# wonheeML/mtl-ssl

Hardware: AMD Instinct MI355X
Metric: images/sec training, Faster R-CNN ResNet-101 + aux heads (higher is better)
Workload: dtype f32; 1 GPU; Faster R-CNN ResNet-101 + window/closeness/edgemask heads + refine, synthetic 1024x600 COCO-shaped (90 classes), per-GPU batch 2 (BASELINE.json configs[1]); global_batch=2, parallelism=dp1, pipeline_config=configs/frcnn_resnet101_coco_mtl.config

## Files before the change

### include/mtlssl_hip.h

```cpp
#ifndef MTLSSL_HIP_H_
#define MTLSSL_HIP_H_

#include <stdint.h>

#ifdef __cplusplus
extern "C" {
#endif

typedef void* mtlssl_stream_t;

#define MTLSSL_OK 0
#define MTLSSL_EINVAL (-1)
#define MTLSSL_ELAUNCH (-2)
#define MTLSSL_ECOMM (-3)

#define MTLSSL_ABI_VERSION 23

const char* mtlssl_last_error(void);
int mtlssl_abi_version(void);

int mtlssl_exp_rn(const double* x, double* y, int64_t n, mtlssl_stream_t stream);

typedef struct {
  int32_t N, H, W, C;
  int32_t K, R, S;
  int32_t OH, OW;
  int32_t stride, dilation;
  int32_t pad_t, pad_l;
  int32_t ldy;
} mtlssl_conv_desc;

#define MTLSSL_EPI_BIAS 1
#define MTLSSL_EPI_RESIDUAL 2
#define MTLSSL_EPI_RELU 4
#define MTLSSL_EPI_TANH 8
#define MTLSSL_EPI_RELU6 16
#define MTLSSL_EPI_MASK 32
#define MTLSSL_EPI_ACCUM 64
#define MTLSSL_EPI_MASK6 128

int64_t mtlssl_conv2d_workspace_bytes(const mtlssl_conv_desc* d, int mode);
int mtlssl_conv2d_fwd(const mtlssl_conv_desc* d, const float* x, const float* w,
                      const float* bias, const float* residual, float* y, int epilogue,
                      void* workspace, mtlssl_stream_t stream);
int mtlssl_conv2d_dgrad(const mtlssl_conv_desc* d, const float* dy, const float* w,
                        const float* residual, const float* mask_ref, float* dx, int epilogue,
                        void* workspace, mtlssl_stream_t stream);
int64_t mtlssl_conv2d_filter_xf_bytes(const mtlssl_conv_desc* d, int mode);
int mtlssl_conv2d_filter_xf_variant(const mtlssl_conv_desc* d, int mode);
// ... 18 lines not shown
typedef struct {
  const float* w;
  float* y;
  const float* bias;
  int32_t K, ldy, epilogue, reserved;
} mtlssl_conv_group_entry;
int mtlssl_conv2d_fwd_grouped(const mtlssl_conv_desc* d, const float* x, int n, const mtlssl_conv_group_entry* entries,
                              int max_k, int sum_k, mtlssl_stream_t stream);
typedef struct {
  const float* dy;
  const float* w;
  int32_t K, ldy;
} mtlssl_conv_seg_entry;
int mtlssl_conv2d_dgrad_segmented(const mtlssl_conv_desc* d, int n, const mtlssl_conv_seg_entry* entries,
                                  const float* residual, const float* mask_ref, float* dx, int epilogue,
                                  mtlssl_stream_t stream);
int mtlssl_conv2d_wgrad_ex(const mtlssl_conv_desc* d, const float* x, const float* dy,
                           const float* out_scale, float* dw, float* dbias, const float* dbias_scale, float beta,
                           void* workspace, const float* input_xf, int input_variant, mtlssl_stream_t stream);
int64_t mtlssl_conv2d_wgrad_workspace_bytes(const mtlssl_conv_desc* d);
int mtlssl_conv2d_tile_config(const mtlssl_conv_desc* d, int mode);
int mtlssl_conv2d_force_config(const mtlssl_conv_desc* d, int mode, int cfg);
int mtlssl_conv2d_set_winograd(int mode);
int mtlssl_conv2d_set_pointwise(int on);
int mtlssl_conv2d_dgrad_rs(const mtlssl_conv_desc* d, const float* dy, const float* w, const float* residual,
                           const float* mask_ref, float* dx, int epilogue, void* workspace, const float* filter_xf,
                           int xf_variant, const uint8_t* group_active, int rows_per_group, mtlssl_stream_t stream);
int mtlssl_conv2d_wgrad_rs(const mtlssl_conv_desc* d, const float* x, const float* dy,
                           const float* out_scale, float* dw, float* dbias, const float* dbias_scale, float beta,
                           void* workspace, const float* input_xf, int input_variant, const uint8_t* group_active,
                           int rows_per_group, mtlssl_stream_t stream);
int mtlssl_row_group_flags(const float* scale, int n, uint8_t* flags, mtlssl_stream_t stream);
int mtlssl_conv2d_set_row_skip(int on);
int mtlssl_conv2d_set_fp32_engine(int mode);
int mtlssl_conv2d_engine_launches(int64_t* out, int reset);
int mtlssl_conv2d_num_dispatches(const mtlssl_conv_desc* d, int mode);
#define MTLSSL_PLAN_INFO_LEN 16
#define MTLSSL_PLAN_DIRECT 0
#define MTLSSL_PLAN_PADDED 1
#define MTLSSL_PLAN_THIN 2
#define MTLSSL_PLAN_S2D 3
#define MTLSSL_PLAN_PARITY 4
#define MTLSSL_PLAN_WINO_F43 5
#define MTLSSL_PLAN_WINO_M7 6
#define MTLSSL_PLAN_VALU 7
int mtlssl_conv2d_plan_info(const mtlssl_conv_desc* d, int mode, int parity_class, int32_t* out);
int64_t mtlssl_conv2d_executed_macs(const mtlssl_conv_desc* d, int mode, int on_mfma);
int mtlssl_conv2d_wgrad(const mtlssl_conv_desc* d, const float* x, const float* dy,
                        const float* out_scale, float* dw, float* dbias, float beta,
                        void* workspace, mtlssl_stream_t stream);

int64_t mtlssl_conv2d_wgrad_grouped_workspace_bytes(const mtlssl_conv_desc* d, int n);
int mtlssl_conv2d_wgrad_grouped(const mtlssl_conv_desc* d, int n, const void* x_ptrs, const void* dy_ptrs,
                                const void* scale_ptrs, const void* dw_ptrs, float beta, void* workspace,
                                mtlssl_stream_t stream);

int mtlssl_depthwise_fwd(const mtlssl_conv_desc* d, const float* x, const float* w, const float* bias,
                         float* y, int epilogue, mtlssl_stream_t stream);
int mtlssl_depthwise_dgrad(const mtlssl_conv_desc* d, const float* dy, const float* w,
                           const float* mask_ref, float* dx, int epilogue, mtlssl_stream_t stream);
int64_t mtlssl_depthwise_wgrad_workspace_bytes(const mtlssl_conv_desc* d);
int mtlssl_depthwise_wgrad(const mtlssl_conv_desc* d, const float* x, const float* dy,
                           const float* out_scale, float* dw, float beta, void* workspace,
                           mtlssl_stream_t stream);
int64_t mtlssl_bn_param_grads_workspace_bytes(int C);
int mtlssl_bn_param_grads(const float* y, const float* g, const float* gamma, const float* beta,
// ... 285 lines not shown
```

### mtl_ssl_amd/build.py

```python
import hashlib
import os
import subprocess
import sys
from concurrent.futures import ThreadPoolExecutor

HERE = os.path.dirname(os.path.abspath(__file__))
CSRC = os.path.join(HERE, "csrc")
OUT = os.path.join(HERE, "libmtlssl_hip.so")
OBJ = os.path.join(HERE, "build")
HIPCC = os.environ.get("HIPCC", "/opt/rocm/bin/hipcc")
COMMON = ["--offload-arch=gfx950", "-O3", "-std=c++17", "-fPIC", "-Wno-unused-result"]
SOURCES = {
    "detection.hip": ["-ffp-contract=off"],
    "ops.hip": ["-ffp-contract=off"],
    "conv.hip": [],
    "glue.hip": ["-ffp-contract=off"],
    "depthwise.hip": [], "pool_concat.hip": [], "winograd.hip": [],
    "eval_metrics.hip": ["-ffp-contract=off"],
    "coco_eval.hip": ["-ffp-contract=off"],
    "pascal_eval.hip": ["-ffp-contract=off"],
    "aux_labels.hip": ["-ffp-contract=off"],
    "summaries.hip": ["-ffp-contract=off"],
    "batch_norm.hip": ["-ffp-contract=off", "-fhip-fp32-correctly-rounded-divide-sqrt"],
    "visualize.hip": [],
    "comm.hip": [],
}


def _digest(path, flags):
    h = hashlib.sha256()
    for f in (path, os.path.join(CSRC, "common.h"), os.path.join(CSRC, "conv_mfma.h"), os.path.join(CSRC, "conv_split.h"), os.path.join(CSRC, "portable_math.h"),
              os.path.join(HERE, "..", "include", "mtlssl_hip.h")):
        with open(f, "rb") as fh:
            h.update(fh.read())
    h.update(" ".join(flags).encode())
    return h.hexdigest()


def build(force=False, verbose=True):
    os.makedirs(OBJ, exist_ok=True)
    jobs, digests = [], []
    for src, extra in SOURCES.items():
        path = os.path.join(CSRC, src)
        obj = os.path.join(OBJ, src + ".o")
        stamp = obj + ".sha"
        dig = _digest(path, COMMON + extra)
        digests.append(dig)
        if (not force and os.path.exists(obj) and os.path.exists(stamp)
                and open(stamp).read() == dig):
            continue
        jobs.append((path, obj, stamp, dig, extra))
    link_stamp = os.path.join(OBJ, "link.sha")
    link_dig = hashlib.sha256("\n".join(digests).encode()).hexdigest()
    if not force and os.path.exists(OUT) and os.path.exists(link_stamp) and open(link_stamp).read() == link_dig:
        return OUT

    def run(job):
        path, obj, stamp, dig, extra = job
        cmd = [HIPCC] + COMMON + extra + ["-c", path, "-o", obj]
        if verbose:
            print(" ".join(cmd), flush=True)
        subprocess.check_call(cmd)
        with open(stamp, "w") as f:
            f.write(dig)
# ... 18 lines not shown
```

### mtl_ssl_amd/csrc/conv.hip

```cpp
#include <stdlib.h>

#include <atomic>
#include <mutex>
#include <unordered_map>

#include "conv_mfma.h"
#include "conv_split.h"

namespace mtlssl {

__global__ void __launch_bounds__(256) k_row_group_flags(const float* __restrict__ scale, int n, uint8_t* __restrict__ flags) {
  const int i = blockIdx.x * blockDim.x + threadIdx.x;
  if (i < n) flags[i] = scale[i] != 0.f;
}
__global__ void __launch_bounds__(256) k_active_ksteps(const uint8_t* __restrict__ flags, int rpg, int P, int pps, int stride,
                                                       int* __restrict__ out) {
  const int z = blockIdx.x, pix0 = z * pps, pix1 = min(P, pix0 + pps);
  const int ksteps = (max(pix1 - pix0, 0) + BK - 1) / BK;
  const int lane = threadIdx.x & 63, w = threadIdx.x >> 6;
  int* list = out + KSTEP_HDR + (int64_t)z * stride;
  __shared__ int wave_cnt[4];
  int base = 0;
  for (int s0 = 0; s0 < ksteps; s0 += 256) {
    const int s = s0 + threadIdx.x;
    bool act = false;
    if (s < ksteps) {
      const int r0 = pix0 + s * BK, r1 = min(r0 + BK, pix1) - 1;
      for (int g = r0 / rpg; g <= r1 / rpg; ++g) act |= flags[g] != 0;
    }
    const unsigned long long m = __ballot(act);
    if (lane == 0) wave_cnt[w] = __popcll(m);
    __syncthreads();
    int off = base;
    for (int i = 0; i < w; ++i) off += wave_cnt[i];
    if (act) list[off + __popcll(m & ((1ull << lane) - 1ull))] = s;
    base += wave_cnt[0] + wave_cnt[1] + wave_cnt[2] + wave_cnt[3];
    __syncthreads();
  }
  if (threadIdx.x == 0) out[z] = base;
}
static inline int64_t kstep_list_bytes(int64_t P) { return align_up((KSTEP_HDR + 2 * cdiv(P, BK) + 128) * 4, 256); }
static std::atomic<int>& row_skip_ref() { static std::atomic<int> v{1}; return v; }

__global__ void __launch_bounds__(256) k_wgrad_reduce(const float* ws, int nsplit, int64_t total4, int K,
                                                      const float* scale, float* dw, float beta, int main_blocks,
                                                      const float* cs_part, int cs_chunks, float* dbias,
                                                      const float* dbias_scale) {
  if ((int)blockIdx.x >= main_blocks) {
    const int lane = threadIdx.x & 63;
    const int k = ((int)blockIdx.x - main_blocks) * 4 + (threadIdx.x >> 6);
    if (k >= K) return;
    float s = 0.f;
    for (int c = lane; c < cs_chunks; c += 64) s += cs_part[(int64_t)c * K + k];
    s = wave_sum(s);
    if (dbias_scale) s *= dbias_scale[k];
    if (lane == 0) dbias[k] = beta != 0.f ? beta * dbias[k] + s : s;
    return;
  }
  const int64_t t = blockIdx.x * (int64_t)blockDim.x + threadIdx.x;
  const int64_t i = t >> 2;
  const int sl = (int)(t & 3);
  const bool live = i < total4;
  floatx4 s = {0.f, 0.f, 0.f, 0.f};
  if (live)
    for (int k = sl; k < nsplit; k += 4) s += reinterpret_cast<const floatx4*>(ws)[(int64_t)k * total4 + i];
#pragma unroll
  for (int e = 0; e < 4; ++e) {
    s[e] += __shfl_xor(s[e], 1, 64);
    s[e] += __shfl_xor(s[e], 2, 64);
  }
  if (!live || sl) return;
  if (scale) s *= *reinterpret_cast<const floatx4*>(scale + (i * 4) % K);
  floatx4* d = reinterpret_cast<floatx4*>(dw) + i;
  *d = beta != 0.f ? beta * *d + s : s;
}
// ... 1227 lines not shown
      (void)hipMemsetAsync(w_pad + (int64_t)d->C * d->K, 0, (size_t)(q.C - d->C) * d->K * 4, S(stream));
      launch_packed<MODE_FWD>(r, p, x_pad, w_pad, workspace, S(stream));
      break;
    }
    case FAM_THIN:
      hipLaunchKernelGGL(k_pw_thin_fwd, dim3(cdiv(p.M, 4)), dim3(256), 0, S(stream), x, w, bias, residual, y, p.M, d->C, d->K, epi);
      break;
    case FAM_GEMM_SMALL: {
      GemmArgs g{x, w, y, bias, residual, nullptr, p.M, d->K, d->C, epi, 0};
      hipLaunchKernelGGL(k_gemm_small<GM_FWD>, dim3(cdiv(g.N, 64), cdiv(g.M, 64)), dim3(256), 0, S(stream), g);
      break;
    }
    case FAM_S2D: {
      float* xs = (float*)workspace;
      float* wsf = (float*)((char*)workspace + r.front_a);
      hipLaunchKernelGGL(k_s2d_pack, dim3(cdiv((int64_t)q.N * q.H * q.W * 4, 256)), dim3(256), 0, S(stream), x, d->N, d->H, d->W,
                         d->C, d->pad_t, d->pad_l, q.H, q.W, xs);
      hipLaunchKernelGGL(k_s2d_filter, dim3(cdiv((int64_t)q.R * q.S * q.C * q.K, 256)), dim3(256), 0, S(stream), w, d->R, d->S,
                         d->C, d->K, q.R, q.S, wsf);
      launch_packed<MODE_FWD>(r, p, xs, wsf, workspace, S(stream));
      break;
    }
    case FAM_STEM_FWD: {
      dim3 grid(cdiv(d->OW, STEM_T), cdiv(d->OH, STEM_T), d->N);
      hipLaunchKernelGGL(k_conv_smallc_fwd, grid, dim3(256), stem_lds_bytes(d), S(stream), p);
      break;
    }
    default:
      hipLaunchKernelGGL(k_conv_direct_fwd, dim3(cdiv((int64_t)p.M * p.K, 256)), dim3(256), 0, S(stream), p);
  }
  return check_launch("conv2d_fwd");
}

int mtlssl_conv2d_fwd_grouped(const mtlssl_conv_desc* d, const float* x, int n, const mtlssl_conv_group_entry* entries,
                              int max_k, int sum_k, mtlssl_stream_t stream) {
  if (n <= 0) return MTLSSL_OK;
  if (int rc = check_desc(d)) return rc;
  MTLSSL_REQUIRE(is_pointwise(d) && d->dilation == 1, "fwd_grouped: pointwise problems only (1x1, stride 1, no padding)");
  MTLSSL_REQUIRE(d->C % BK == 0, "fwd_grouped: C = %d must be a multiple of %d", d->C, BK);
  MTLSSL_REQUIRE(x && entries && n <= MTLSSL_CONV_GROUP_MAX && max_k >= 16 && sum_k >= max_k, "fwd_grouped: bad arguments");
  ConvArgs p = make_args(d);
  GroupArgs ga;
  memset(&ga, 0, sizeof(ga));
  p.a = x;
  for (int i = 0; i < n; ++i) {
    const mtlssl_conv_group_entry& e = entries[i];
    MTLSSL_REQUIRE(e.w && e.y && e.K >= 16 && e.K % 4 == 0 && e.K <= max_k && (e.ldy == 0 || (e.ldy >= e.K && e.ldy % 4 == 0)) &&
                       !(e.epilogue & (MTLSSL_EPI_RESIDUAL | MASK_ANY | MTLSSL_EPI_ACCUM)) && (!(e.epilogue & MTLSSL_EPI_BIAS) || e.bias),
                   "fwd_grouped: problem %d: K = %d, ldy = %d, epilogue = %d", i, e.K, e.ldy, e.epilogue);
    ga.e[i] = e;
  }
  p.a_bytes = (unsigned)((int64_t)d->N * d->H * d->W * d->C * 4);
  p.M = d->N * d->H * d->W;
  p.NG = max_k; p.K = max_k; p.ldy = 0;
  p.nsplit = 1; p.ks_per_split = 0; p.tile_m0 = 0; p.ws_m0 = 0;
  int cfg = 2;
  double best = 1e30;
  for (int c = 0; c < NCFG; ++c) {
    const int64_t tiles = cdiv(p.M, CFG_BM[c]) * cdiv(sum_k, CFG_BN[c]);
    const double t = tile_time_us(c, tiles, d->C / CFG_BK[c], true);
    if (t < best) { best = t; cfg = c; }
  }
  p.tiles_m = (int)cdiv(p.M, CFG_BM[cfg]);
  p.tiles_n = (int)cdiv(max_k, CFG_BN[cfg]);
  dim3 grid(p.tiles_m * p.tiles_n, n, 1);
  count_engine_launch(0);
// ... 448 lines not shown
```

### mtl_ssl_amd/frcnn.py

```python
import os

import torch

from . import nn, ops

f32, i32 = torch.float32, torch.int32


def _init_from_hyperparams(hp):
    ini = hp.initializer
    which = ini.which_oneof(["truncated_normal_initializer", "variance_scaling_initializer"])
    if which == "truncated_normal_initializer":
        return ("truncated_normal", float(ini.truncated_normal_initializer.stddev))
    if which == "variance_scaling_initializer":
        v = ini.variance_scaling_initializer
        return ("variance_scaling", float(v.factor), str(v.mode), bool(v.uniform))
    return ("variance_scaling", 1.0, "FAN_AVG", True)


def _l2_from_hyperparams(hp):
    reg = hp.regularizer
    if reg.has("l2_regularizer"):
        return float(reg.l2_regularizer.weight)
    return 0.0
# ... 32 lines not shown
        if not self.spatial_average:
            if feat_hw is None:
                raise ValueError("mask_rcnn_box_predictor without spatial_average needs the tower's output size")
            width = cin * int(feat_hw[0]) * int(feat_hw[1])
        depth = max(min(cin, int(cfg.max_depth)), int(cfg.min_depth))
        self.stack = None
        n_extra = int(cfg.num_layers_before_predictor) if depth > 0 else 0
        if n_extra > 0:
            act = {"RELU": "relu", "NONE": None}.get(str(cfg.fc_hyperparams.activation))
            if act is None and str(cfg.fc_hyperparams.activation) != "NONE":
                raise ValueError("fc_hyperparams.activation %s is not supported in the predictor's extra layers"
                                 % cfg.fc_hyperparams.activation)
            self.stack = nn.FCStack(ps, ["%s/FC_%d_%d" % (scope, i, depth) for i in range(n_extra)], width,
                                    [depth] * n_extra, init, is_training, wd, activation=act,
                                    keep_prob=float(cfg.dropout_keep_probability) if cfg.use_dropout else None,
                                    slot0=slot0, batch_norm=bn)
            width = depth
        self.box = None
        if not class_only:
            self.box = nn.Conv(ps, scope + "/BoxEncodingPredictor", width, num_classes * 4, 1, init,
                               is_training, wd, fc=True, batch_norm=bn and bn())
            self.cls = nn.Conv(ps, scope + "/ClassPredictor", width, num_classes + 1, 1, init, is_training,
                               wd, fc=True, batch_norm=bn and bn())
        else:
            self.cls = nn.Conv(ps, scope + "/ClassPredictor", width, num_classes, 1, init, is_training, wd,
                               fc=True, batch_norm=bn and bn())

    def layers(self):
        extra = self.stack.layers if self.stack is not None else []
        return extra + [l for l in (self.box, self.cls) if l is not None]

    def predict(self, feat, seed=0, step=0, update=False):
        pooled = ops.spatial_mean_fwd(feat) if self.spatial_average else feat.reshape(feat.shape[0], -1)
        net, sctx = pooled, None
        if self.stack is not None:
            net, sctx = self.stack.forward(pooled, self.is_training, seed, step, update)
        out = {"pooled": net, "_stack_ctx": sctx}
        for key, head in (("class", self.cls), ("box", self.box)):
            if head is not None and head.batch_stats:
                keep = out["_norm_" + key] = {}
                out[key] = head.forward(net, keep, update)
            elif head is not None:
                out[key] = head.forward(net)
        return out

    def backward(self, pred, d_class, d_box, feat_shape, need_feat_grad=True, mask_ref=None, mask6=False):
        net = pred["pooled"]
        if self.cls.norm is not None:
            d_class = self.cls.norm_backward(pred.get("_norm_class"), pred["class"], d_class)
            if d_box is not None:
                d_box = self.box.norm_backward(pred.get("_norm_box"), pred["box"], d_box)
        self.cls.wgrad(net, d_class)
        if d_box is not None:
            self.box.wgrad(net, d_box)
        if not need_feat_grad and self.stack is None:
            return None
        dp = self.cls.dgrad(net.shape, d_class)
        if d_box is not None:
            self.box.dgrad(net.shape, d_box, out=dp, accum=True)
        if self.stack is not None:
            dp = self.stack.backward(pred["_stack_ctx"], dp, need_input_grad=need_feat_grad)
        if not need_feat_grad:
            return None
        if self.spatial_average:
            return ops.spatial_mean_bwd(dp, feat_shape, mask_ref, mask6)
        g = dp.reshape(tuple(feat_shape))
# ... 431 lines not shown
        stop = bool(self._mtl.stop_gradient_for_aux_tasks)
        need_crop_grad = not stop
        crops, argmax = self._crop(F, flat, box_ind, need_crop_grad)
        save = self._is_training and not (self._shared_classifier and stop)
        feat, ctx = self.window_tower.forward(crops, save)
        wp = self.window_predictor.predict(feat, self.seed, self.step)
        pd.update({"window_class_predictions": wp["class"], "_wfeat": feat, "_wctx": ctx, "_wp": wp,
                   "_wcrops": crops, "_wargmax": argmax, "_wboxes": flat, "_wbox_ind": box_ind})
        return pd

    def predict_edgemask(self, pd):
        pd["edgemask_predictions"] = self.edgemask_conv.forward(pd["rpn_features_to_crop"])
        return pd

    DEDUP_SLOTS = 8

    def check_device_flags(self):
        f = self._dedup_overflow
        if f is not None and int(f.item()) != 0:
            raise RuntimeError("refiner window de-duplication overflowed its %d slots per image (non-finite or "
                               "out-of-range proposal boxes?)" % self.DEDUP_SLOTS)

    def _refine_window_predictions(self, F, boxes_norm):
        B = F.shape[0]
        N2 = self.max_num_proposals
        K1 = self.num_classes + 1
        ew = ops.expand_windows(boxes_norm, self.N_EXPAND)
        if self.DEDUP_SLOTS > 0:
            if self._dedup_overflow is None:
                self._dedup_overflow = torch.zeros((1,), dtype=torch.int32, device=F.device)
            rois, src_row = ops.dedup_windows(ew, self.DEDUP_SLOTS, self._dedup_overflow)
            R = rois.shape[1]
            crops, _ = self._crop(F, rois.view(B * R, 4), self._box_ind(B, R, F.device), False)
            feat, _ = self.window_tower.forward(crops, False)
            compact = self.window_predictor.predict(feat, self.seed, self.step)["class"]
            return ops.gather_rows(compact.view(1, B * R, K1), src_row)
        flat = ew.view(B * self.N_EXPAND * N2, 4)
        crops, _ = self._crop(F, flat, self._box_ind(B, self.N_EXPAND * N2, F.device), False)
        feat, _ = self.window_tower.forward(crops, False)
        return self.window_predictor.predict(feat, self.seed, self.step)["class"]

    def _refine_stream(self):
        if self._aux_stream() is None or os.environ.get("MTLSSL_REFINE_EARLY", "0") != "1":
            return None
        return self._wgrad_exec().stream

    def _expand_window_class_predictions(self, pd):
        if "_refine_win" in pd:
            ops.wait_on(self._refine_stream(), "refine: early window pass")
            win = pd.pop("_refine_win")
            win.record_stream(torch.cuda.current_stream())
            return win
        return self._refine_window_predictions(pd["rpn_features_to_crop"], pd["proposal_boxes_normalized"])

    def predict_with_mtl_results(self, pd):
        mtl = self._mtl
        B = pd["rpn_features_to_crop"].shape[0]
        N2 = self.max_num_proposals
        K1 = self.num_classes + 1
        cls = pd["class_predictions_with_background"]
        win = None
        if mtl.window:
            win = self._expand_window_class_predictions(pd)
            pd["expand_window_class_predictions"] = win.view(B, self.N_EXPAND, N2, K1)
        clo = pd["closeness_predictions"] if mtl.closeness else None
        net = ops.refine_concat(cls, win, clo, B, N2, self.N_EXPAND, bool(mtl.global_closeness))
        hidden, sctx = net, None
        if self.refine_stack is not None:
            hidden, sctx = self.refine_stack.forward(net, self._is_training, self.seed, self.step)
        refined = self.refine_fc.forward(hidden)
        pd["_refine_hidden"], pd["_refine_ctx"] = hidden, sctx
        if mtl.refine_residue:
            ops.axpby(cls, refined, 1.0, 1.0)
# ... 320 lines not shown
```

### mtl_ssl_amd/lib.py

```python
import ctypes
import os
import re

HERE = os.path.dirname(os.path.abspath(__file__))
HEADER = os.path.join(HERE, "..", "include", "mtlssl_hip.h")
LIB_PATH = os.environ.get("MTLSSL_LIB_PATH") or os.path.join(HERE, "libmtlssl_hip.so")


class ConvDesc(ctypes.Structure):
    _fields_ = [(n, ctypes.c_int32) for n in
                ("N", "H", "W", "C", "K", "R", "S", "OH", "OW", "stride", "dilation",
                 "pad_t", "pad_l", "ldy")]


_SCALARS = {
    "int": ctypes.c_int, "int32_t": ctypes.c_int32, "int64_t": ctypes.c_int64,
    "uint32_t": ctypes.c_uint32, "float": ctypes.c_float, "double": ctypes.c_double,
    "mtlssl_stream_t": ctypes.c_void_p, "mtlssl_comm_t": ctypes.c_void_p,
}


def _ctype(decl):
    decl = decl.strip()
    if "*" in decl:
# ... 17 lines not shown
            for a in args.split(","):
                a = a.strip()
                a = re.sub(r"\s*\w+$", "", a) if not a.endswith("*") else a
                argtypes.append(_ctype(a))
        protos[name] = (restype, argtypes)
    return protos


class MtlsslError(RuntimeError):
    pass


class _Lib:
    def __init__(self):
        if not os.path.exists(LIB_PATH):
            raise MtlsslError(
                "%s not found: build it with `python -m mtl_ssl_amd.build` "
                "(there is no CPU fallback for the product path)" % LIB_PATH)
        import torch
        self.cdll = ctypes.CDLL(LIB_PATH)
        self.protos = parse_header()
        want = int(re.search(r"#define\s+MTLSSL_ABI_VERSION\s+(\d+)", open(HEADER).read()).group(1))
        self.cdll.mtlssl_abi_version.restype = ctypes.c_int
        have = self.cdll.mtlssl_abi_version()
        if have != want:
            raise MtlsslError("%s has ABI version %d, include/mtlssl_hip.h declares %d: rebuild it with "
                              "`python -m mtl_ssl_amd.build`" % (LIB_PATH, have, want))
        for name, (restype, argtypes) in self.protos.items():
            fn = getattr(self.cdll, name)
            fn.restype = restype
            fn.argtypes = argtypes
            if restype is ctypes.c_int and name not in ("mtlssl_abi_version", "mtlssl_conv2d_tile_config", "mtlssl_conv2d_num_dispatches",
                                                        "mtlssl_conv2d_set_winograd", "mtlssl_conv2d_set_fp32_engine", "mtlssl_conv2d_filter_xf_variant",
                                                        "mtlssl_conv2d_set_pointwise", "mtlssl_conv2d_set_row_skip"):
                setattr(self, name[len("mtlssl_"):], self._checked(fn, name))
            else:
                setattr(self, name[len("mtlssl_"):], fn)

    def _checked(self, fn, name):
        last_error = self.cdll.mtlssl_last_error

        def call(*args):
            rc = fn(*args)
            if rc != 0:
                raise MtlsslError("%s failed (%d): %s" % (name, rc, last_error().decode()))
        return call


_lib = None


def lib():
    global _lib
    if _lib is None:
        _lib = _Lib()
    return _lib


def ptr(t):
    return None if t is None else t.data_ptr()
```

### mtl_ssl_amd/nn.py

```python
import torch

from . import ops

f32 = torch.float32


def _refresh_bn(layer):
    if layer.bn_trainable:
        ps = layer.ps
        if layer.gamma is not None:
            torch.mul(ps.value(layer.gamma.name), layer.inv_std, out=layer.scale)
        torch.addcmul(ps.value(layer.beta.name), ps.value(layer.mean.name), layer.scale, value=-1.0,
                      out=layer.shift)


class WgradStream:

    def __init__(self, stream):
        self.stream = stream

    def run(self, layer, x, g, **kw):
        if not layer.trainable:
            return
        ev = torch.cuda.Event()
# ... 94 lines not shown
            ops.bn_param_grads(y, gp, ps.value(self.gamma.name), ps.value(self.beta.name),
                               ps.grad(self.gamma.name), ps.grad(self.beta.name), beta=1.0)
            ps.grad_ready(self.gamma, self.beta)


class ConvBN(_FrozenBN):

    def __init__(self, ps, scope, cin, cout, k, stride=1, dilation=1, padding="SAME",
                 trainable=True, weight_decay=0.0, eps=1e-5, gamma_init=1.0, relu=True, act=None,
                 init=("variance_scaling", 2.0, "FAN_IN", False), bn_trainable=False,
                 weights_name="weights", bn_scale=True):
        super().__init__()
        self.ps, self.scope = ps, scope
        self.bn_trainable = bn_trainable
        self.k, self.stride, self.dilation, self.padding, self.eps = k, stride, dilation, padding, eps
        self.trainable = trainable
        self.act = act if act is not None else ("relu" if relu else None)
        self.relu = self.act is not None
        kh, kw = k if isinstance(k, tuple) else (k, k)
        self.w = ps.add(scope + "/" + weights_name, (kh, kw, cin, cout), init, trainable, weight_decay)
        self.w_eff_shape = self.w.shape
        self._add_batch_norm(cout, gamma_init, bn_scale)
        self._kept = {}

    def geometry(self):
        return self.w.shape, self.stride, self.dilation, self.padding

    def forward(self, x, residual=None, relu=None, keep=False, out=None):
        act = self.act if relu is None else ("relu" if relu else None)
        epi = ops.EPI_BIAS | act_epilogue(act) | (ops.EPI_RESIDUAL if residual is not None else 0)
        return ops.conv2d_fwd(self.desc(x.shape), x, self.w_eff, self.shift, residual, epi, out=out,
                              xf_cache=self.ps.filter_cache,
                              keep_input_xf=self._keep_slot() if (keep and self.trainable and self.k == 3) else None)

    def _keep_slot(self):
        if len(self._kept) > 8:
            self._kept.clear()
        return self._kept

    def wgrad(self, x, g, active=None):
        if self.trainable:
            db = self.ps.grad(self.beta.name) if (self.bn_trainable and self.gamma is None) else None
            ops.conv2d_wgrad(self.desc(x.shape), x, g, self.ps.grad(self.w.name), out_scale=self.scale,
                             dbias=db, beta=1.0, input_xf=self._kept.pop(x.data_ptr(), None), active=active)
            self.ps.grad_ready(self.w, self.beta if db is not None else None)

    def dgrad(self, x_shape, g, residual=None, mask_ref=None, out=None, accum=False, mask6=False, active=None):
        return ops.conv2d_dgrad(self.desc(x_shape), g, self.w_eff, residual, mask_ref,
                                dgrad_epilogue(residual, accum, mask_ref, mask6), out=out, xf_cache=self.ps.filter_cache,
                                active=active)


class DepthwiseBN(_FrozenBN):

    def __init__(self, ps, scope, c, k=3, stride=1, dilation=1, trainable=True, weight_decay=0.0, eps=1e-3,
                 act="relu6", init=("truncated_normal", 0.09), bn_trainable=False, gamma_init=1.0, batch_norm=True):
        super().__init__()
        self.ps, self.scope, self.c = ps, scope, c
        self.bn_trainable = bn_trainable
        self.k, self.stride, self.dilation, self.eps, self.act = k, stride, dilation, eps, act
        self.trainable = trainable
        self.w = ps.add(scope + "/depthwise_weights", (k, k, c, 1), init, trainable, weight_decay)
        self.w_eff_shape = (k, k, c)
        if batch_norm:
            self._add_batch_norm(c, gamma_init)

# ... 233 lines not shown
                 weight_decay=0.0, bn_trainable=False):
        s = scope + "/bottleneck_v1/"
        self.stride, self.cin, self.depth = stride, cin, depth
        self.shortcut = None
        if depth != cin:
            self.shortcut = ConvBN(ps, s + "shortcut", cin, depth, 1, stride, 1, "SAME", trainable,
                                   weight_decay, relu=False, bn_trainable=bn_trainable)
        self.conv1 = ConvBN(ps, s + "conv1", cin, depth_bottleneck, 1, 1, 1, "SAME", trainable, weight_decay,
                            bn_trainable=bn_trainable)
        self.conv2 = ConvBN(ps, s + "conv2", depth_bottleneck, depth_bottleneck, 3, stride, rate,
                            "RESNET_SAME", trainable, weight_decay, bn_trainable=bn_trainable)
        self.conv3 = ConvBN(ps, s + "conv3", depth_bottleneck, depth, 1, 1, 1, "SAME", trainable,
                            weight_decay, gamma_init=0.3, relu=True, bn_trainable=bn_trainable)
        self.trainable = trainable
        self.bn_trainable = bn_trainable

    def layers(self):
        return [l for l in (self.shortcut, self.conv1, self.conv2, self.conv3) if l is not None]

    def forward(self, x, save):
        if self.shortcut is not None:
            sc = self.shortcut.forward(x)
        elif self.stride > 1:
            sc, _ = ops.maxpool_fwd(x, 1, self.stride, "SAME")
        else:
            sc = x
        a1 = self.conv1.forward(x)
        a2 = self.conv2.forward(a1, keep=save)
        out = self.conv3.forward(a2, residual=sc)
        ctx = (x, a1, a2, sc if (self.shortcut is None and self.stride > 1) else None) if save else None
        if save and self.bn_trainable:
            ctx = ctx + (out, sc)
        return out, ctx

    def backward(self, gp, ctx, need_input_grad=True, mask_input=True, wgrad=INLINE_WGRAD, active=None):
        kw = {} if active is None else dict(active=active)
        x, a1, a2, sc_sub = ctx[:4]
        if self.bn_trainable:
            out, sc = ctx[4], ctx[5]
            o3 = ops.axpby(sc, out.clone(), -1.0, 1.0)
            self.conv3.bn_grad(o3, gp)
            del o3
            if self.shortcut is not None:
                self.shortcut.bn_grad(sc, gp)
        wgrad.run(self.conv3, a2, gp, **kw)
        gp2 = self.conv3.dgrad(a2.shape, gp, mask_ref=a2, **kw)
        if self.bn_trainable:
            self.conv2.bn_grad(a2, gp2)
        wgrad.run(self.conv2, a1, gp2, **kw)
        gp1 = self.conv2.dgrad(a1.shape, gp2, mask_ref=a1, **kw)
        if self.bn_trainable:
            self.conv1.bn_grad(a1, gp1)
        wgrad.run(self.conv1, x, gp1, **kw)
        if self.shortcut is not None:
            wgrad.run(self.shortcut, x, gp, **kw)
        if not need_input_grad:
            return None
        if self.shortcut is not None:
            addend = self.shortcut.dgrad(x.shape, gp, **kw)
        elif self.stride > 1:
            addend = ops.maxpool_bwd(x, sc_sub, gp, 1, self.stride, (0, 0))
        else:
            addend = gp
        return self.conv1.dgrad(x.shape, gp1, residual=addend, mask_ref=x if mask_input else None, **kw)


# ... 69 lines not shown
```

### mtl_ssl_amd/ops.py

```python
import ctypes
import os

import numpy as np
import torch

from .lib import ConvDesc, lib, ptr

EPI_BIAS, EPI_RESIDUAL, EPI_RELU, EPI_TANH, EPI_RELU6, EPI_MASK, EPI_ACCUM, EPI_MASK6 = 1, 2, 4, 8, 16, 32, 64, 128
f32 = torch.float32
i32 = torch.int32


_raw_stream = getattr(torch._C, "_cuda_getCurrentRawStream", None)
_cur_device = getattr(torch._C, "_cuda_getDevice", None)


def _stream():
    if _raw_stream is not None and _cur_device is not None:
        return _raw_stream(_cur_device())
    return torch.cuda.current_stream().cuda_stream


def _chk(t, dtype=f32):
    assert t.is_cuda and t.is_contiguous() and t.dtype == dtype, (t.device, t.dtype, t.is_contiguous())
    return t


def _chk_y(d, t):
    if not d.ldy:
        return _chk(t)
    assert t.is_cuda and t.dtype == f32 and t.dim() == 4 and t.shape[-1] == d.K and t.stride(-1) == 1 \
        and t.stride(-2) == d.ldy and t.stride(-3) == d.ldy * t.shape[-2] and t.data_ptr() % 16 == 0, \
        (tuple(t.shape), t.stride(), d.ldy)
    return t


_ws_cache = {}


# ... 446 lines not shown
def _conv_ws(d, mode, device):
    nb = lib().conv2d_workspace_bytes(ctypes.byref(d), mode)
    return workspace(nb, "wgrad" if mode == 2 else "splitk", device) if nb else None


def conv2d_fwd(d, x, w, bias=None, residual=None, epilogue=0, out=None, xf_cache=None, keep_input_xf=None):
    if d.ldy:
        assert out is not None, "a strided forward writes into the caller's concatenated map"
        _chk_y(d, out)
    y = out if out is not None else torch.empty((d.N, d.OH, d.OW, d.K), dtype=f32, device=x.device)
    if PROFILER is None:
        def run():
            lib().conv2d_fwd(ctypes.byref(d), ptr(_chk(x)), ptr(_chk(w)), ptr(bias), ptr(residual), ptr(y), epilogue,
                             ptr(_conv_ws(d, 0, x.device)), _stream())
        _autotune(d, 0, run)
    t0 = PROFILER.begin(d, 0) if PROFILER is not None else None
    if ACCOUNT is not None:
        ACCOUNT.add(d, 0)
    ws = _conv_ws(d, 0, x.device)
    U, variant = xf_cache.get(d, 0, w) if (xf_cache is not None and d.R == 3 and d.S == 3) else (None, -1)
    V, vvar = None, -1
    if keep_input_xf is not None:
        vvar = _shared_input_variant(d)
        if vvar >= 0:
            V = torch.empty(int(lib().conv2d_input_xf_bytes(ctypes.byref(d), vvar)) // 4, dtype=f32, device=x.device)
            keep_input_xf[x.data_ptr()] = (V, vvar)
    lib().conv2d_fwd_keep(ctypes.byref(d), ptr(_chk(x)), ptr(_chk(w)), ptr(bias), ptr(residual),
                          ptr(y), epilogue, ptr(ws), ptr(U), variant, ptr(V), vvar, _stream())
    if t0 is not None:
        PROFILER.end(d, 0, t0)
    return y


def set_row_skip(on):
    return lib().conv2d_set_row_skip(int(on))


def row_group_flags(scale):
    flags = torch.empty(scale.numel(), dtype=torch.uint8, device=scale.device)
    lib().row_group_flags(ptr(_chk(scale)), scale.numel(), ptr(flags), _stream())
    return flags


def _active_arg(d, active, rows=None):
    if active is None:
        return None, 0
    assert active.dtype == torch.uint8 and active.is_contiguous() and active.numel() == d.N, (active.dtype, active.shape, d.N)
    return ptr(active), rows if rows is not None else d.OH * d.OW


def conv2d_dgrad(d, dy, w, residual=None, mask_ref=None, epilogue=0, out=None, xf_cache=None, active=None):
    dx = out if out is not None else torch.empty((d.N, d.H, d.W, d.C), dtype=f32, device=dy.device)
    if PROFILER is None:
        def run():
            tmp = workspace(4 * d.N * d.H * d.W * d.C, "tune_out", dy.device)
            lib().conv2d_dgrad(ctypes.byref(d), ptr(_chk_y(d, dy)), ptr(_chk(w)), ptr(residual), ptr(mask_ref), ptr(tmp),
                               epilogue & ~EPI_ACCUM, ptr(_conv_ws(d, 1, dy.device)), _stream())
        _autotune(d, 1, run)
    t0 = PROFILER.begin(d, 1) if PROFILER is not None else None
    if ACCOUNT is not None:
        ACCOUNT.add(d, 1)
    ws = _conv_ws(d, 1, dy.device)
    U, variant = xf_cache.get(d, 1, w) if (xf_cache is not None and d.R == 3 and d.S == 3) else (None, -1)
    lib().conv2d_dgrad_rs(ctypes.byref(d), ptr(_chk_y(d, dy)), ptr(_chk(w)), ptr(residual), ptr(mask_ref),
                          ptr(dx), epilogue, ptr(ws), ptr(U), variant, *_active_arg(d, active, d.H * d.W), _stream())
    if t0 is not None:
# ... 1003 lines not shown
```

### mtl_ssl_amd/resnet.py

```python
import torch

from . import nn, ops

RESNET_UNITS = {"resnet_v1_50": (3, 4, 6, 3), "resnet_v1_101": (3, 4, 23, 3),
                "resnet_v1_152": (3, 8, 36, 3)}


class BoxClassifierTower(nn.Tower):
    out_act = "relu"
    supports_wgrad_stream = True

    def __init__(self, ps, scope, arch, cin, trainable, weight_decay, bn_trainable=False):
        self.stack = nn.BlockStack(ps, "%s/%s" % (scope, arch), cin,
                                   [("block4", 512, 3, 1, trainable)], None, 1, weight_decay, bn_trainable)
        self.trainable = trainable
        self.cout = self.stack.cout

    def layers(self):
        return self.stack.layers()

    def forward(self, crops, save):
        x, ctxs = crops, []
        for u in self.stack.units:
            x, c = u.forward(x, save)
            ctxs.append(c)
        return x, (ctxs if save else None)

    def backward(self, g_out, out, ctxs, need_input_grad, masked=False, wgrad=nn.INLINE_WGRAD, active=None):
        gp = g_out if masked else ops.relu_bwd(out, g_out)
        units = self.stack.units
        for i in range(len(units) - 1, -1, -1):
            first = i == 0
            gp = units[i].backward(gp, ctxs[i], need_input_grad=(need_input_grad or not first),
                                   mask_input=not first, wgrad=wgrad, active=active)
        return gp


class FasterRCNNResnetV1FeatureExtractor(nn.FeatureExtractor):
    channel_means = (123.68, 116.779, 103.939)
    out_act = "relu"
    supports_wgrad_stream = True

    def __init__(self, ps, architecture, is_training, first_stage_features_stride=16,
                 weight_decay=0.0, freeze_layer="block1", batch_norm_trainable=False,
                 first_stage_scope="FirstStageFeatureExtractor"):
        super().__init__(ps, is_training, first_stage_features_stride, weight_decay)
        self.bn_trainable = bool(batch_norm_trainable) and bool(is_training)
        self.arch = architecture
        n_freeze = int(freeze_layer[-1]) if freeze_layer else 0
        bt = [False] * n_freeze + [bool(is_training)] * (4 - n_freeze)
        units = RESNET_UNITS[architecture]
        prefix = "%s/%s" % (first_stage_scope, architecture)
        self.conv1 = nn.ConvBN(ps, prefix + "/conv1", 3, 64, 7, 2, 1, "RESNET_SAME", False, weight_decay,
                               gamma_init=0.015, bn_trainable=self.bn_trainable)
        blocks = [("block1", 64, units[0], 2, bt[0]), ("block2", 128, units[1], 2, bt[1]),
                  ("block3", 256, units[2], 2, bt[2])]
        self.trunk = nn.BlockStack(ps, prefix, 64, blocks, first_stage_features_stride // 4, 1, weight_decay,
                                   self.bn_trainable)
        self.cout = self.trunk.cout
# ... 40 lines not shown
```

Baseline: 41.70 images/sec.

## Fuse window tower's last 1x1 conv with spatial mean into a group-mean kernel

Adds a pointwise MFMA conv kernel whose epilogue applies bias, residual and activation, then sums rows per spatial group into per-tile partials, followed by a small finish kernel that writes per-crop channel means. The forward-only window-prediction path uses it for the last bottleneck unit instead of materializing the full output and then running a separate spatial mean. This avoids writing and re-reading the large final feature map, at the cost of an extra launch and a partials workspace. It is guarded by a runtime toggle that defaults on.

```diff
diff --git a/include/mtlssl_hip.h b/include/mtlssl_hip.h
--- a/include/mtlssl_hip.h
+++ b/include/mtlssl_hip.h
@@ -14,7 +14,7 @@
 #define MTLSSL_ELAUNCH (-2)
 #define MTLSSL_ECOMM (-3)
 
-#define MTLSSL_ABI_VERSION 23
+#define MTLSSL_ABI_VERSION 24
 
 const char* mtlssl_last_error(void);
 int mtlssl_abi_version(void);
@@ -99,6 +99,11 @@
                            int rows_per_group, mtlssl_stream_t stream);
 int mtlssl_row_group_flags(const float* scale, int n, uint8_t* flags, mtlssl_stream_t stream);
 int mtlssl_conv2d_set_row_skip(int on);
+int64_t mtlssl_conv2d_fwd_groupmean_partial_bytes(const mtlssl_conv_desc* d, int rows_per_group);
+int mtlssl_conv2d_fwd_groupmean(const mtlssl_conv_desc* d, const float* x, const float* w, const float* bias,
+                                const float* residual, float* mean, int epilogue, int rows_per_group, void* partials,
+                                mtlssl_stream_t stream);
+int mtlssl_set_window_fusion(int on);
 int mtlssl_conv2d_set_fp32_engine(int mode);
 int mtlssl_conv2d_engine_launches(int64_t* out, int reset);
 int mtlssl_conv2d_num_dispatches(const mtlssl_conv_desc* d, int mode);
diff --git a/mtl_ssl_amd/build.py b/mtl_ssl_amd/build.py
--- a/mtl_ssl_amd/build.py
+++ b/mtl_ssl_amd/build.py
@@ -29,7 +29,7 @@
 
 def _digest(path, flags):
     h = hashlib.sha256()
-    for f in (path, os.path.join(CSRC, "common.h"), os.path.join(CSRC, "conv_mfma.h"), os.path.join(CSRC, "conv_split.h"), os.path.join(CSRC, "portable_math.h"),
+    for f in (path, os.path.join(CSRC, "common.h"), os.path.join(CSRC, "conv_mfma.h"), os.path.join(CSRC, "conv_groupmean.h"), os.path.join(CSRC, "conv_split.h"), os.path.join(CSRC, "portable_math.h"),
               os.path.join(HERE, "..", "include", "mtlssl_hip.h")):
         with open(f, "rb") as fh:
             h.update(fh.read())
diff --git a/mtl_ssl_amd/csrc/conv.hip b/mtl_ssl_amd/csrc/conv.hip
--- a/mtl_ssl_amd/csrc/conv.hip
+++ b/mtl_ssl_amd/csrc/conv.hip
@@ -4,6 +4,7 @@
 #include <mutex>
 #include <unordered_map>
 
+#include "conv_groupmean.h"
 #include "conv_mfma.h"
 #include "conv_split.h"
 
@@ -41,6 +42,7 @@
 }
 static inline int64_t kstep_list_bytes(int64_t P) { return align_up((KSTEP_HDR + 2 * cdiv(P, BK) + 128) * 4, 256); }
 static std::atomic<int>& row_skip_ref() { static std::atomic<int> v{1}; return v; }
+static std::atomic<int>& window_fusion_ref() { static std::atomic<int> v{1}; return v; }
 
 __global__ void __launch_bounds__(256) k_wgrad_reduce(const float* ws, int nsplit, int64_t total4, int K,
                                                       const float* scale, float* dw, float beta, int main_blocks,
@@ -1334,6 +1336,71 @@
   return check_launch("conv2d_fwd");
 }
 
+static int groupmean_check(const mtlssl_conv_desc* d, int rows_per_group) {
+  if (int rc = check_desc(d)) return rc;
+  MTLSSL_REQUIRE(is_pointwise(d) && d->dilation == 1, "fwd_groupmean: pointwise problems only (1x1, stride 1, no padding)");
+  MTLSSL_REQUIRE(d->C % BK == 0 && d->K >= 16 && d->K % 4 == 0, "fwd_groupmean: C = %d must be a multiple of %d, K = %d a multiple of 4 and >= 16",
+                 d->C, BK, d->K);
+  MTLSSL_REQUIRE(desc_dense(d), "fwd_groupmean: no output map, so no ldy (%d)", d->ldy);
+  const int64_t M = (int64_t)d->N * d->H * d->W;
+  MTLSSL_REQUIRE(rows_per_group >= 32 && M % rows_per_group == 0, "fwd_groupmean: rows_per_group = %d must be >= 32 and divide the %lld rows",
+                 rows_per_group, (long long)M);
+  return MTLSSL_OK;
+}
+static int groupmean_tile(const mtlssl_conv_desc* d) {
+  const Route r = route(d, MODE_FWD);
+  return r.family == FAM_DIRECT ? r.plan.cfg % NCFG : -1;
+}
+
+int64_t mtlssl_conv2d_fwd_groupmean_partial_bytes(const mtlssl_conv_desc* d, int rows_per_group) {
+  if (!d || groupmean_check(d, rows_per_group)) return 0;
+  const int cfg = groupmean_tile(d);
+  if (cfg < 0) return 0;
+  const int64_t M = (int64_t)d->N * d->H * d->W;
+  return align_up(cdiv(M, CFG_BM[cfg]) * gm_nseg(CFG_BM[cfg], rows_per_group) * d->K * 4, 256);
+}
+
+int mtlssl_conv2d_fwd_groupmean(const mtlssl_conv_desc* d, const float* x, const float* w, const float* bias,
+                                const float* residual, float* mean, int epi, int rows_per_group, void* partials,
+                                mtlssl_stream_t stream) {
+  if (int rc = groupmean_check(d, rows_per_group)) return rc;
+  MTLSSL_REQUIRE(x && w && mean && partials, "fwd_groupmean: null pointer");
+  MTLSSL_REQUIRE(!(epi & MTLSSL_EPI_BIAS) || bias, "fwd_groupmean: bias pointer required");
+  MTLSSL_REQUIRE(!(epi & MTLSSL_EPI_RESIDUAL) || residual, "fwd_groupmean: residual pointer required");
+  MTLSSL_REQUIRE(!(epi & (MASK_ANY | MTLSSL_EPI_ACCUM)), "fwd_groupmean: forward epilogue flags only (%d)", epi);
+  const int cfg = groupmean_tile(d);
+  MTLSSL_REQUIRE(cfg >= 0, "fwd_groupmean: the problem is not planned on the tile engine");
+  ConvArgs p = make_args(d);
+  p.a = x; p.b = w; p.out = (float*)partials; p.bias = bias; p.residual = residual; p.epi = epi;
+  p.a_bytes = (unsigned)((int64_t)d->N * d->H * d->W * d->C * 4);
+  p.b_bytes = (unsigned)((int64_t)d->C * d->K * 4);
+  p.M = d->N * d->H * d->W;
+  p.NG = d->K;
+  p.nsplit = 1;
+  p.rows_per_group = rows_per_group;
+  p.tiles_m = (int)cdiv(p.M, CFG_BM[cfg]);
+  p.tiles_n = (int)cdiv(p.NG, CFG_BN[cfg]);
+  const int nseg = gm_nseg(CFG_BM[cfg], rows_per_group);
+  const dim3 grid(p.tiles_m * p.tiles_n);
+  count_engine_launch(0);
+  switch (cfg) {
+    case 0: hipLaunchKernelGGL((k_conv_pw_gmean<128, 128>), grid, dim3(256), 0, S(stream), p, nseg); break;
+    case 1: hipLaunchKernelGGL((k_conv_pw_gmean<128, 64>), grid, dim3(256), 0, S(stream), p, nseg); break;
+    case 2: hipLaunchKernelGGL((k_conv_pw_gmean<64, 64>), grid, dim3(256), 0, S(stream), p, nseg); break;
+    default: hipLaunchKernelGGL((k_conv_pw_gmean<256, 128>), grid, dim3(512), 0, S(stream), p, nseg); break;
+  }
+  const int groups = p.M / rows_per_group;
+  hipLaunchKernelGGL(k_groupmean_finish, dim3(cdiv((int64_t)groups * (d->K / 4), 256)), dim3(256), 0, S(stream),
+                     (const float*)partials, mean, groups, d->K / 4, rows_per_group, CFG_BM[cfg], nseg);
+  return check_launch("conv2d_fwd_groupmean");
+}
+
+int mtlssl_set_window_fusion(int on) {
+  const int prev = window_fusion_ref().load();
+  if (on == 0 || on == 1) window_fusion_ref().store(on);
+  return prev;
+}
+
 int mtlssl_conv2d_fwd_grouped(const mtlssl_conv_desc* d, const float* x, int n, const mtlssl_conv_group_entry* entries,
                               int max_k, int sum_k, mtlssl_stream_t stream) {
   if (n <= 0) return MTLSSL_OK;
diff --git a/mtl_ssl_amd/csrc/conv_groupmean.h b/mtl_ssl_amd/csrc/conv_groupmean.h
--- /dev/null
+++ b/mtl_ssl_amd/csrc/conv_groupmean.h
@@ -0,0 +1,217 @@
+#pragma once
+#include "conv_mfma.h"
+
+namespace mtlssl {
+
+constexpr int gm_max_segs(int bm) { return bm / 32 + 1; }
+static inline int gm_nseg(int bm, int rpg) {
+  const int n = (bm - 1) / rpg + 2;
+  return n < gm_max_segs(bm) ? n : gm_max_segs(bm);
+}
+
+template <int BM, int BN>
+__global__ void __launch_bounds__(BM > 128 ? 512 : 256, (BM > 128 ? 2 : BM * BN >= 128 * 128 ? 3 : 4))
+k_conv_pw_gmean(ConvArgs p, int nseg) {
+  constexpr int BKT = BK;
+  constexpr int NW = BM > 128 ? 8 : 4, NT = 64 * NW, WR = NW / 2;
+  constexpr int LDA = BM + 4, LDB = BN + 4;
+  constexpr int KQ = BKT / 4, RP = NT / KQ;
+  constexpr int TM = BM / (32 * WR), TN = BN / 64;
+  constexpr int A_LD = BM / RP, B_LD = BN / RP;
+  constexpr unsigned OOB = 0xFFFFFFF0u;
+  constexpr int LDT = 36, SEGS = gm_max_segs(BM);
+  constexpr int SMEM_OPS = 2 * BKT * (LDA + LDB), SMEM_EPI = NW * 32 * LDT + WR * SEGS * BN;
+  __shared__ __attribute__((aligned(16))) float smem[SMEM_OPS > SMEM_EPI ? SMEM_OPS : SMEM_EPI];
+  float* const sA = smem;
+  float* const sB = smem + 2 * BKT * LDA;
+
+  const int nwg = p.tiles_m * p.tiles_n;
+  int bid = blockIdx.x;
+  {
+    int q = nwg / 8, r = nwg % 8, xcd = bid % 8, loc = bid / 8;
+    bid = (xcd < r ? xcd * (q + 1) : r * (q + 1) + (xcd - r) * q) + loc;
+  }
+  const int tile_m = bid / p.tiles_n, tile_n = bid % p.tiles_n;
+  const int m0 = tile_m * BM, n0 = tile_n * BN;
+  const int tid = threadIdx.x, lane = tid & 63, wid = tid >> 6;
+  const int wr = wid >> 1, wc = wid & 1;
+  const int lo = lane & 31, hi = lane >> 5;
+  const int kq4 = (tid % KQ) * 4;
+  const int nk = p.C / BKT;
+
+  __amdgpu_buffer_rsrc_t rsrc_a = __builtin_amdgcn_make_buffer_rsrc(const_cast<float*>(p.a), 0, p.a_bytes, 0x00020000);
+  __amdgpu_buffer_rsrc_t rsrc_b = __builtin_amdgcn_make_buffer_rsrc(const_cast<float*>(p.b), 0, p.b_bytes, 0x00020000);
+  unsigned a_voff[A_LD], b_base[B_LD];
+#pragma unroll
+  for (int i = 0; i < A_LD; ++i) {
+    const int m = m0 + (tid / KQ) + RP * i;
+    a_voff[i] = m < p.M ? (unsigned)(m * p.C + kq4) * 4u : OOB;
+  }
+#pragma unroll
+  for (int i = 0; i < B_LD; ++i) {
+    const int u = tid + NT * i;
+    const int col = n0 + (u % (BN / 4)) * 4;
+    b_base[i] = col < p.NG ? (unsigned)((u / (BN / 4)) * p.K + col) * 4u : OOB;
+  }
+
+  floatx4 rA[2][A_LD], rB[2][B_LD];
+  using Set0 = std::integral_constant<int, 0>;
+  using Set1 = std::integral_constant<int, 1>;
+  auto load_tile = [&](int ks, auto SET) {
+    floatx4 (&ra)[A_LD] = rA[decltype(SET)::value];
+    floatx4 (&rb)[B_LD] = rB[decltype(SET)::value];
+    const unsigned ka = (unsigned)(ks * BKT) * 4u, so = (unsigned)(ks * BKT * p.K) * 4u;
+#pragma unroll
+    for (int i = 0; i < A_LD; ++i) ra[i] = bufload4(rsrc_a, a_voff[i], ka);
+#pragma unroll
+    for (int i = 0; i < B_LD; ++i) rb[i] = bufload4(rsrc_b, b_base[i], so);
+  };
+  auto store_tile = [&](int buf, auto SET) {
+    floatx4 (&ra)[A_LD] = rA[decltype(SET)::value];
+    floatx4 (&rb)[B_LD] = rB[decltype(SET)::value];
+    float* a = sA + buf * (BKT * LDA);
+    float* b = sB + buf * (BKT * LDB);
+#pragma unroll
+    for (int i = 0; i < A_LD; ++i) {
+      const int row = (tid / KQ) + RP * i;
+      a[(kq4 + 0) * LDA + row] = ra[i].x; a[(kq4 + 1) * LDA + row] = ra[i].y;
+      a[(kq4 + 2) * LDA + row] = ra[i].z; a[(kq4 + 3) * LDA + row] = ra[i].w;
+    }
+#pragma unroll
+    for (int i = 0; i < B_LD; ++i) {
+      const int u = tid + NT * i;
+      *reinterpret_cast<floatx4*>(b + (u / (BN / 4)) * LDB + (u % (BN / 4)) * 4) = rb[i];
+    }
+  };
+
+  floatx16 acc[TM][TN];
+#pragma unroll
+  for (int i = 0; i < TM; ++i)
+#pragma unroll
+    for (int j = 0; j < TN; ++j)
+#pragma unroll
+      for (int e = 0; e < 16; ++e) acc[i][j][e] = 0.f;
+
+  if (nk > 0) {
+    load_tile(0, Set0{});
+    store_tile(0, Set0{});
+  }
+  if (nk > 1) load_tile(1, Set1{});
+  __syncthreads();
+  auto kstep = [&](int it, auto next, auto spare) {
+    const int cur = it & 1;
+    if (it + 2 < nk) load_tile(it + 2, spare);
+    const float* a = sA + cur * (BKT * LDA) + wr * (BM / WR) + lo;
+    const float* b = sB + cur * (BKT * LDB) + wc * (BN / 2) + lo;
+    float fa[2][TM], fb[2][TN];
+#pragma unroll
+    for (int i = 0; i < TM; ++i) fa[0][i] = a[hi * LDA + i * 32];
+#pragma unroll
+    for (int j = 0; j < TN; ++j) fb[0][j] = b[hi * LDB + j * 32];
+#pragma unroll
+    for (int kk = 0; kk < BKT / 2; ++kk) {
+      const int cs = kk & 1, ns = cs ^ 1;
+      if (kk + 1 < BKT / 2) {
+        const int kr = 2 * (kk + 1) + hi;
+#pragma unroll
+        for (int i = 0; i < TM; ++i) fa[ns][i] = a[kr * LDA + i * 32];
+#pragma unroll
+        for (int j = 0; j < TN; ++j) fb[ns][j] = b[kr * LDB + j * 32];
+      }
+      __builtin_amdgcn_sched_barrier(0);
+#pragma unroll
+      for (int i = 0; i < TM; ++i)
+#pragma unroll
+        for (int j = 0; j < TN; ++j)
+          acc[i][j] = __builtin_amdgcn_mfma_f32_32x32x2f32(fa[cs][i], fb[cs][j], acc[i][j], 0, 0, 0);
+      __builtin_amdgcn_sched_barrier(0);
+    }
+    if (it + 1 < nk) store_tile(cur ^ 1, next);
+    __syncthreads();
+  };
+  for (int it = 0; it < nk; it += 2) {
+    kstep(it, Set1{}, Set0{});
+    if (it + 1 < nk) kstep(it + 1, Set0{}, Set1{});
+  }
+
+  float* tile = smem + wid * (32 * LDT);
+  float* part = smem + NW * 32 * LDT;
+  const int rpg = p.rows_per_group;
+  const int g0 = m0 / rpg;
+  if (hi == 0) {
+#pragma unroll
+    for (int s = 0; s < SEGS; ++s)
+#pragma unroll
+      for (int j = 0; j < TN; ++j) part[(wr * SEGS + s) * BN + wc * (BN / 2) + j * 32 + lo] = 0.f;
+  }
+  const int r_in = lane >> 3, c4 = (lane & 7) * 4;
+#pragma unroll
+  for (int i = 0; i < TM; ++i) {
+#pragma unroll
+    for (int j = 0; j < TN; ++j) {
+#pragma unroll
+      for (int e = 0; e < 16; ++e) tile[((e & 3) + 8 * (e >> 2) + 4 * hi) * LDT + lo] = acc[i][j][e];
+      const int cw = wc * (BN / 2) + j * 32;
+      const int col = n0 + cw + c4;
+      const int rbase = m0 + wr * (BM / WR) + i * 32;
+      floatx4 bv = {0.f, 0.f, 0.f, 0.f};
+      if ((p.epi & MTLSSL_EPI_BIAS) && col < p.NG) bv = *reinterpret_cast<const floatx4*>(p.bias + col);
+#pragma unroll
+      for (int k = 0; k < 4; ++k) {
+        const int rt = r_in + 8 * k;
+        const int row = rbase + rt;
+        floatx4 v = *reinterpret_cast<const floatx4*>(tile + rt * LDT + c4);
+        if (row < p.M && col < p.NG) {
+          v += bv;
+          if (p.epi & MTLSSL_EPI_RESIDUAL) v += *reinterpret_cast<const floatx4*>(p.residual + (int64_t)row * p.NG + col);
+#pragma unroll
+          for (int q = 0; q < 4; ++q) {
+            if (p.epi & MTLSSL_EPI_RELU) v[q] = fmaxf(v[q], 0.f);
+            if (p.epi & MTLSSL_EPI_RELU6) v[q] = fminf(fmaxf(v[q], 0.f), 6.f);
+            if (p.epi & MTLSSL_EPI_TANH) v[q] = tanhf(v[q]);
+          }
+        } else {
+          v = floatx4{0.f, 0.f, 0.f, 0.f};
+        }
+        *reinterpret_cast<floatx4*>(tile + rt * LDT + c4) = v;
+      }
+      if (hi == 0) {
+        const int rend = min(rbase + 32, p.M);
+        int row = rbase;
+        while (row < rend) {
+          const int g = row / rpg;
+          const int stop = min(rend, (g + 1) * rpg);
+          float s = 0.f;
+          for (; row < stop; ++row) s += tile[(row - rbase) * LDT + lo];
+          part[(wr * SEGS + (g - g0)) * BN + cw + lo] += s;
+        }
+      }
+    }
+  }
+  __syncthreads();
+  const int nseg_here = (min(m0 + BM, p.M) - 1) / rpg - g0 + 1;
+  for (int u = tid; u < nseg_here * BN; u += NT) {
+    const int s = u / BN, c = u % BN;
+    float t = part[s * BN + c];
+#pragma unroll
+    for (int w = 1; w < WR; ++w) t += part[(w * SEGS + s) * BN + c];
+    if (n0 + c < p.NG) p.out[((int64_t)tile_m * nseg + s) * p.NG + n0 + c] = t;
+  }
+}
+
+__global__ void __launch_bounds__(256) k_groupmean_finish(const float* __restrict__ part, float* __restrict__ mean,
+                                                          int groups, int K4, int rpg, int bm, int nseg) {
+  const int64_t idx = (int64_t)blockIdx.x * blockDim.x + threadIdx.x;
+  if (idx >= (int64_t)groups * K4) return;
+  const int g = (int)(idx / K4), c = (int)(idx % K4);
+  const int t0 = g * rpg / bm, t1 = ((g + 1) * rpg - 1) / bm;
+  floatx4 s = {0.f, 0.f, 0.f, 0.f};
+  for (int t = t0; t <= t1; ++t) {
+    const int seg = g - t * bm / rpg;
+    s += reinterpret_cast<const floatx4*>(part)[((int64_t)t * nseg + seg) * K4 + c];
+  }
+  const float n = (float)rpg;
+  reinterpret_cast<floatx4*>(mean)[idx] = floatx4{s[0] / n, s[1] / n, s[2] / n, s[3] / n};
+}
+
+}
diff --git a/mtl_ssl_amd/frcnn.py b/mtl_ssl_amd/frcnn.py
--- a/mtl_ssl_amd/frcnn.py
+++ b/mtl_ssl_amd/frcnn.py
@@ -88,6 +88,9 @@
 
     def predict(self, feat, seed=0, step=0, update=False):
         pooled = ops.spatial_mean_fwd(feat) if self.spatial_average else feat.reshape(feat.shape[0], -1)
+        return self.predict_from_mean(pooled, seed, step, update)
+
+    def predict_from_mean(self, pooled, seed=0, step=0, update=False):
         net, sctx = pooled, None
         if self.stack is not None:
             net, sctx = self.stack.forward(pooled, self.is_training, seed, step, update)
@@ -585,13 +588,19 @@
             rois, src_row = ops.dedup_windows(ew, self.DEDUP_SLOTS, self._dedup_overflow)
             R = rois.shape[1]
             crops, _ = self._crop(F, rois.view(B * R, 4), self._box_ind(B, R, F.device), False)
-            feat, _ = self.window_tower.forward(crops, False)
-            compact = self.window_predictor.predict(feat, self.seed, self.step)["class"]
+            compact = self._window_predictions_forward_only(crops)
             return ops.gather_rows(compact.view(1, B * R, K1), src_row)
         flat = ew.view(B * self.N_EXPAND * N2, 4)
         crops, _ = self._crop(F, flat, self._box_ind(B, self.N_EXPAND * N2, F.device), False)
-        feat, _ = self.window_tower.forward(crops, False)
-        return self.window_predictor.predict(feat, self.seed, self.step)["class"]
+        return self._window_predictions_forward_only(crops)
+
+    def _window_predictions_forward_only(self, crops):
+        tower, pred = self.window_tower, self.window_predictor
+        if (pred.spatial_average and hasattr(tower, "forward_mean") and crops.shape[1] * crops.shape[2] >= 32
+                and ops.set_window_fusion(-1) == 1):
+            return pred.predict_from_mean(tower.forward_mean(crops), self.seed, self.step)["class"]
+        feat, _ = tower.forward(crops, False)
+        return pred.predict(feat, self.seed, self.step)["class"]
 
     def _refine_stream(self):
         if self._aux_stream() is None or os.environ.get("MTLSSL_REFINE_EARLY", "0") != "1":
diff --git a/mtl_ssl_amd/lib.py b/mtl_ssl_amd/lib.py
--- a/mtl_ssl_amd/lib.py
+++ b/mtl_ssl_amd/lib.py
@@ -73,7 +73,7 @@
             fn.argtypes = argtypes
             if restype is ctypes.c_int and name not in ("mtlssl_abi_version", "mtlssl_conv2d_tile_config", "mtlssl_conv2d_num_dispatches",
                                                         "mtlssl_conv2d_set_winograd", "mtlssl_conv2d_set_fp32_engine", "mtlssl_conv2d_filter_xf_variant",
-                                                        "mtlssl_conv2d_set_pointwise", "mtlssl_conv2d_set_row_skip"):
+                                                        "mtlssl_conv2d_set_pointwise", "mtlssl_conv2d_set_row_skip", "mtlssl_set_window_fusion"):
                 setattr(self, name[len("mtlssl_"):], self._checked(fn, name))
             else:
                 setattr(self, name[len("mtlssl_"):], fn)
diff --git a/mtl_ssl_amd/nn.py b/mtl_ssl_amd/nn.py
--- a/mtl_ssl_amd/nn.py
+++ b/mtl_ssl_amd/nn.py
@@ -150,6 +150,10 @@
         return ops.conv2d_fwd(self.desc(x.shape), x, self.w_eff, self.shift, residual, epi, out=out,
                               xf_cache=self.ps.filter_cache,
                               keep_input_xf=self._keep_slot() if (keep and self.trainable and self.k == 3) else None)
+
+    def forward_mean(self, x, residual=None):
+        epi = ops.EPI_BIAS | act_epilogue(self.act) | (ops.EPI_RESIDUAL if residual is not None else 0)
+        return ops.conv2d_fwd_groupmean(self.desc(x.shape), x, self.w_eff, self.shift, residual, epi)
 
     def _keep_slot(self):
         if len(self._kept) > 8:
@@ -449,6 +453,12 @@
         if save and self.bn_trainable:
             ctx = ctx + (out, sc)
         return out, ctx
+
+    def forward_mean(self, x):
+        assert self.stride == 1
+        sc = self.shortcut.forward(x) if self.shortcut is not None else x
+        a2 = self.conv2.forward(self.conv1.forward(x))
+        return self.conv3.forward_mean(a2, residual=sc)
 
     def backward(self, gp, ctx, need_input_grad=True, mask_input=True, wgrad=INLINE_WGRAD, active=None):
         kw = {} if active is None else dict(active=active)
diff --git a/mtl_ssl_amd/ops.py b/mtl_ssl_amd/ops.py
--- a/mtl_ssl_amd/ops.py
+++ b/mtl_ssl_amd/ops.py
@@ -4,7 +4,7 @@
 import numpy as np
 import torch
 
-from .lib import ConvDesc, lib, ptr
+from .lib import ConvDesc, MtlsslError, lib, ptr
 
 EPI_BIAS, EPI_RESIDUAL, EPI_RELU, EPI_TANH, EPI_RELU6, EPI_MASK, EPI_ACCUM, EPI_MASK6 = 1, 2, 4, 8, 16, 32, 64, 128
 f32 = torch.float32
@@ -517,6 +517,27 @@
     return y
 
 
+def conv2d_fwd_groupmean(d, x, w, bias=None, residual=None, epilogue=0, rows_per_group=None):
+    rpg = int(rows_per_group) if rows_per_group else d.H * d.W
+    nb = int(lib().conv2d_fwd_groupmean_partial_bytes(ctypes.byref(d), rpg))
+    if not nb:
+        raise MtlsslError("conv2d_fwd_groupmean does not take this problem: %s" % (_plan_key(d, 0),))
+    mean = torch.empty((d.N * d.H * d.W // rpg, d.K), dtype=f32, device=x.device)
+    t0 = PROFILER.begin(d, 0) if PROFILER is not None else None
+    if ACCOUNT is not None:
+        ACCOUNT.add(d, 0)
+    part = workspace(nb, "groupmean", x.device)
+    lib().conv2d_fwd_groupmean(ctypes.byref(d), ptr(_chk(x)), ptr(_chk(w)), ptr(bias), ptr(residual), ptr(mean),
+                               epilogue, rpg, ptr(part), _stream())
+    if t0 is not None:
+        PROFILER.end(d, 0, t0)
+    return mean
+
+
+def set_window_fusion(on):
+    return lib().set_window_fusion(int(on))
+
+
 def set_row_skip(on):
     return lib().conv2d_set_row_skip(int(on))
 
diff --git a/mtl_ssl_amd/resnet.py b/mtl_ssl_amd/resnet.py
--- a/mtl_ssl_amd/resnet.py
+++ b/mtl_ssl_amd/resnet.py
@@ -25,6 +25,12 @@
             x, c = u.forward(x, save)
             ctxs.append(c)
         return x, (ctxs if save else None)
+
+    def forward_mean(self, crops):
+        x = crops
+        for u in self.stack.units[:-1]:
+            x, _ = u.forward(x, False)
+        return self.stack.units[-1].forward_mean(x)
 
     def backward(self, g_out, out, ctxs, need_input_grad, masked=False, wgrad=nn.INLINE_WGRAD, active=None):
         gp = g_out if masked else ops.relu_bwd(out, g_out)
```

Measured after the change: 41.64 images/sec. Within noise of the previous version (-0.1%).
